# templeblock/audioSignalProcess

Hardware: AMD Instinct MI355X
Metric: audio frames/sec (10 ms @16 kHz) Wiener NS (higher is better)
Workload: dtype f32

## Files before the change

### audiosignalprocess_amd/csrc/ns_api.hip

```cpp
#include <hip/hip_runtime.h>

#include <chrono>

#include <math.h>
#include <stdio.h>
#include <stdlib.h>
#include <string.h>

#include <mutex>
#include <vector>

#include "api_common.h"
#include "asp_ns.h"
#include "handoff_host.h"
#include "ns_layout.h"

using namespace aspns;

namespace aspns {
hipError_t launch_ns_frame(int mode, float* state, int32_t* hist, const NsTables* T,
                           const float* in, float* out, int num_streams, hipStream_t s, bool g8 = false);
hipError_t launch_ns_frame1(bool io16, float* state, int32_t* hist, const NsTables* T,
                            const float* in, float* out, int num_streams, hipStream_t s, int steady_on,
                            unsigned long long* stamps = nullptr, int stamp_mode = 0, unsigned* step_counts = nullptr);
// ... 2 lines not shown
                                 unsigned* seq, unsigned* abort_w, unsigned want, int steps, int walk, int slot0,
                                 int ring, size_t per, int steady_on, unsigned long long* stamps = nullptr,
                                 unsigned* step_counts = nullptr);
hipError_t launch_ns_frame2(bool io16, float* state, int32_t* hist, const NsTables* T,
                            const float* in, float* out, int num_streams, hipStream_t s,
                            unsigned long long* stamps = nullptr);
hipError_t launch_ns_frame2_flow(bool io16, float* state, int32_t* hist, const NsTables* T,
                                 const float* in, float* out, int num_streams, hipStream_t s,
                                 unsigned* seq, unsigned* abort_w, unsigned want, int steps, int slot0, int ring,
                                 size_t per, unsigned long long* stamps = nullptr);
hipError_t launch_ns_unpair(float* state, int num_streams, hipStream_t s);
hipError_t launch_ns_hb_live(const float* state, const NsTables* T, const float* in_low,
                             int32_t* live, int num_streams, int hist_off, hipStream_t s);
hipError_t launch_ns_hb_apply(const float* state, float* hb_tail, const int32_t* live,
                              const NsTables* T, const float* in_high, float* out_high,
                              int num_streams, int num_high, int paired, hipStream_t s);
hipError_t launch_ns_set_policy(float* state, int num_streams, int mode, float overdrive,
                                float denoiseBound, int gainmap, hipStream_t s);
hipError_t launch_rdft256(float* data, int count, int isgn, const NsTables* T, hipStream_t s, int n = 256);
hipError_t launch_debug_eval(int fn, float* data, size_t n, const NsTables* T, hipStream_t s);
hipError_t launch_debug_tanh_wave(unsigned start, unsigned count, unsigned* n_bad, unsigned* bad_bits,
                                  const NsTables* T, hipStream_t s);
hipError_t launch_debug_guards_wave(unsigned start, unsigned count, unsigned* n_bad, unsigned* bad_bits, hipStream_t s);
hipError_t launch_debug_compare(int fn_a, int fn_b, unsigned start, unsigned count,
                                unsigned* n_bad, unsigned* bad_bits, float param,
                                const NsTables* T, hipStream_t s);
}

namespace {

#define fail(...) asp_fail(nullptr, __VA_ARGS__)
#define HIP_TRY(x) ASP_TRY(nullptr, x)
constexpr const char* kNoDevice = "no HIP device available (the NS engine has no CPU fallback)";


unsigned bitrev(unsigned x, int bits) {
  unsigned r = 0;
  for (int b = 0; b < bits; ++b) r |= ((x >> b) & 1u) << (bits - 1 - b);
  return r;
}

float window_entry(int i) {
  if (i >= 96 && i <= 160) return 1.0f;
  char buf[32];
  double s = sin(M_PI * (double)(i < 96 ? i : 256 - i) / 192.0);
  snprintf(buf, sizeof buf, "%.8f", s);
// ... 1460 lines not shown
  if (e == hipSuccess) e = hipMemcpy(data, d, n * sizeof(float), hipMemcpyDeviceToHost);
  (void)hipFree(d);
  if (e != hipSuccess) return fail(ASP_ERR_HIP, "debug_eval", e);
  return ASP_OK;
}

int AspNs_debug_compare(int fn_a, int fn_b, uint32_t start, uint32_t count, uint32_t* n_bad,
                        uint32_t* bad_bits64, float param, int device) {
  if (!n_bad || !bad_bits64) return fail(ASP_ERR_PARAM, "debug_compare: bad argument");
  AspDeviceScope dev_scope_;
  int rc = dev_scope_.select(nullptr, device, ASP_ERR_PARAM, kNoDevice);
  if (rc) return rc;
  NsTables* T = nullptr;
  rc = device_tables(device, &T);
  if (rc) return rc;
  unsigned* d = nullptr;
  HIP_TRY(hipMalloc((void**)&d, 65 * sizeof(unsigned)));
  hipError_t e = hipMemset(d, 0, 65 * sizeof(unsigned));
  if (e == hipSuccess && fn_a == 23 && fn_b != 3) e = hipErrorInvalidValue;
  if (e == hipSuccess && fn_a == 24 && fn_b != 9) e = hipErrorInvalidValue;
  if (e == hipSuccess)
    e = fn_a == 23   ? launch_debug_tanh_wave(start, count, d, d + 1, T, nullptr)
        : fn_a == 24 ? launch_debug_guards_wave(start, count, d, d + 1, nullptr)
                     : launch_debug_compare(fn_a, fn_b, start, count, d, d + 1, param, T, nullptr);
  unsigned h[65];
  if (e == hipSuccess) e = hipMemcpy(h, d, sizeof h, hipMemcpyDeviceToHost);
  (void)hipFree(d);
  if (e != hipSuccess) return fail(ASP_ERR_HIP, "debug_compare", e);
  *n_bad = h[0];
  memcpy(bad_bits64, h + 1, 64 * sizeof(unsigned));
  return ASP_OK;
}


struct NsHandleT {
  AspNsBatch* batch;
  int initFlag;
};

int WebRtcNs_Create(NsHandle** NS_inst) {
  if (!NS_inst) return -1;
  NsHandleT* h = (NsHandleT*)malloc(sizeof(NsHandleT));
  if (!h) return -1;
  h->batch = nullptr;
  h->initFlag = 0;
  if (AspNsBatch_Create(&h->batch, 1, 0) != ASP_OK) {
// ... 77 lines not shown
```

### audiosignalprocess_amd/csrc/ns_device.h

```cpp
#pragma once
#include <hip/hip_runtime.h>

namespace aspns_dev {

#ifdef NS1_BUDGET
#define ASP_NS_RARE(c) (__builtin_assume(!(c)), false)
#else
#define ASP_NS_RARE(c) __builtin_expect((c), 0)
#endif

__device__ __forceinline__ float xorf(float x, uint32_t m) {
  return __uint_as_float(__float_as_uint(x) ^ m);
}

__device__ __forceinline__ void wave_lds_fence() {
  __builtin_amdgcn_fence(__ATOMIC_RELEASE, "wavefront");
  __builtin_amdgcn_wave_barrier();
  __builtin_amdgcn_fence(__ATOMIC_ACQUIRE, "wavefront");
}

template <int CTRL>
__device__ __forceinline__ float dpp_move(float v) {
  return __int_as_float(__builtin_amdgcn_update_dpp(0, __float_as_int(v), CTRL, 0xF, 0xF, true));
}
// ... 56 lines not shown
  c = __int_as_float(__builtin_amdgcn_readlane(__float_as_int(c), 63));
  d = __int_as_float(__builtin_amdgcn_readlane(__float_as_int(d), 63));
}

__device__ __forceinline__ float div_by_uniform(float a, float d, float rd) {
  const float q0 = a * rd;
  const float r = __builtin_fmaf(-d, q0, a);
  return __builtin_fmaf(r, rd, q0);
}

__device__ __forceinline__ float fdiv_rcp(float d) {
  const float r0 = __builtin_amdgcn_rcpf(d);
  const float e0 = __builtin_fmaf(-d, r0, 1.0f);
  return __builtin_fmaf(e0, r0, r0);
}
__device__ __forceinline__ float fdiv_quot(float n, float d, float r1) {
  const float q0 = n * r1;
  const float e1 = __builtin_fmaf(-d, q0, n);
  const float q1 = __builtin_fmaf(e1, r1, q0);
  const float e2 = __builtin_fmaf(-d, q1, n);
  return __builtin_fmaf(e2, r1, q1);
}
__device__ __forceinline__ float fdiv(float n, float d) { return fdiv_quot(n, d, fdiv_rcp(d)); }
typedef float f32x2 __attribute__((ext_vector_type(2)));
__device__ __forceinline__ f32x2 fdiv2_rcp(f32x2 d) {
  f32x2 r0;
  r0.x = __builtin_amdgcn_rcpf(d.x);
  r0.y = __builtin_amdgcn_rcpf(d.y);
  const f32x2 one = {1.0f, 1.0f};
  const f32x2 e0 = __builtin_elementwise_fma(-d, r0, one);
  return __builtin_elementwise_fma(e0, r0, r0);
}
__device__ __forceinline__ f32x2 fdiv2_quot(f32x2 n, f32x2 d, f32x2 r1) {
  const f32x2 q0 = n * r1;
  const f32x2 e1 = __builtin_elementwise_fma(-d, q0, n);
  const f32x2 q1 = __builtin_elementwise_fma(e1, r1, q0);
  const f32x2 e2 = __builtin_elementwise_fma(-d, q1, n);
  return __builtin_elementwise_fma(e2, r1, q1);
}
__device__ __forceinline__ f32x2 fdiv2(f32x2 n, f32x2 d) { return fdiv2_quot(n, d, fdiv2_rcp(d)); }
struct B3 {
  bool v[3];
};
struct F3 {
  f32x2 p;
  float t;
  __device__ __forceinline__ F3() {}
  __device__ __forceinline__ F3(f32x2 p_, float t_) : p(p_), t(t_) {}
  __device__ __forceinline__ explicit F3(float c) : p(f32x2{c, c}), t(c) {}
  __device__ __forceinline__ explicit F3(const float (&x)[3]) : p(f32x2{x[0], x[1]}), t(x[2]) {}
  __device__ __forceinline__ void store(float (&x)[3]) const {
    x[0] = p.x; x[1] = p.y; x[2] = t;
  }
};
__device__ __forceinline__ F3 operator+(const F3& x, const F3& y) { return F3(x.p + y.p, x.t + y.t); }
__device__ __forceinline__ F3 operator-(const F3& x, const F3& y) { return F3(x.p - y.p, x.t - y.t); }
__device__ __forceinline__ F3 operator*(const F3& x, const F3& y) { return F3(x.p * y.p, x.t * y.t); }
__device__ __forceinline__ F3 operator*(float c, const F3& y) { return F3(c) * y; }
__device__ __forceinline__ F3 operator*(const F3& x, float c) { return x * F3(c); }
__device__ __forceinline__ F3 operator+(const F3& x, float c) { return x + F3(c); }
__device__ __forceinline__ F3 operator-(const F3& x, float c) { return x - F3(c); }
__device__ __forceinline__ F3 operator-(float c, const F3& y) { return F3(c) - y; }
__device__ __forceinline__ F3 fma3(const F3& x, const F3& y, const F3& z) {
// ... 119 lines not shown
  s = __builtin_fma(s0 * d, d, s);
  const double z = s * s;
  double p = 2.0 / 21.0;
  p = __builtin_fma(p, z, 2.0 / 19.0);
  p = __builtin_fma(p, z, 2.0 / 17.0);
  p = __builtin_fma(p, z, 2.0 / 15.0);
  p = __builtin_fma(p, z, 2.0 / 13.0);
  p = __builtin_fma(p, z, 2.0 / 11.0);
  p = __builtin_fma(p, z, 2.0 / 9.0);
  p = __builtin_fma(p, z, 2.0 / 7.0);
  p = __builtin_fma(p, z, 2.0 / 5.0);
  p = __builtin_fma(p, z, 2.0 / 3.0);
  const double lm = __builtin_fma(s * z, p, s + s);
  const double ed = (double)e;
  const double ln2_hi = 0x1.62e42fefa38p-1;
  const double ln2_lo = 0x1.ef35793c7673p-45;
  return __builtin_fma(ed, ln2_hi, __builtin_fma(ed, ln2_lo, lm));
}

__device__ __forceinline__ bool f64_rounds_safely_to_f32(double y) {
  const unsigned lo = (unsigned)__double2loint(y) & 0x1fffffffu;
  return ((lo - 0x0ffffe00u) > 0x400u);
}

__device__ __forceinline__ double exp_lean_f64(float xf, const double* __restrict__ t64) {
  const double x = (double)xf;
  const double kd = __builtin_rint(x * 0x1.71547652b82fep+6);
  const int k = (int)kd;
  double r = __builtin_fma(-kd, 0x1.62e42ff000000p-7, x);
  r = __builtin_fma(-kd, -0x1.718432a1b0e26p-41, r);
  double q = 1.0 / 120.0;
  q = __builtin_fma(q, r, 1.0 / 24.0);
  q = __builtin_fma(q, r, 1.0 / 6.0);
  q = __builtin_fma(q, r, 0.5);
  const double p = __builtin_fma(q, r * r, r);
  const double T = t64[k & 63];
  return __builtin_amdgcn_ldexp(__builtin_fma(T, p, T), k >> 6);
}

__device__ __forceinline__ float exp_f32_via_f64(float x, const double* __restrict__ t64) {
  const bool in_range = fabsf(x) <= 87.0f;
  const double y = exp_lean_f64(in_range ? x : 0.0f, t64);
  const bool ok = in_range && f64_rounds_safely_to_f32(y);
  float r = (float)y;
  if (ASP_NS_RARE(!ok)) r = (float)exp((double)x);
  return r;
// ... 5 lines not shown
  const double ad = (double)ax;
  const double a2 = ad * ad;
  double sr = 0x1.664f4882c10fap-6;
  sr = __builtin_fma(sr, a2, -0x1.ba1ba1ba1ba1cp-5);
  sr = __builtin_fma(sr, a2, 0x1.1111111111111p-3);
  sr = __builtin_fma(sr, a2, -0x1.5555555555555p-2);
  const double t_small = __builtin_fma(ad * a2, sr, ad);
  const double u = exp_lean_f64(finite_ok ? -2.0f * ax : 0.0f, t64);
  const double num = 1.0 - u, den = 1.0 + u;
  double rc = (double)__builtin_amdgcn_rcpf((float)den);
  rc = __builtin_fma(__builtin_fma(-den, rc, 1.0), rc, rc);
  rc = __builtin_fma(__builtin_fma(-den, rc, 1.0), rc, rc);
  double qv = num * rc;
  qv = __builtin_fma(__builtin_fma(-qv, den, num), rc, qv);
  const double t = ax < 0.03125f ? t_small : qv;
  const bool ok = finite_ok && f64_rounds_safely_to_f32(t);
  float r = __builtin_copysignf((float)t, a);
  if (ASP_NS_RARE(!ok)) r = (float)tanh((double)a);
  return r;
}

__device__ __forceinline__ float tanh_f32_via_f64_wave(float a, const double* __restrict__ t64) {
  const float ax = fabsf(a);
  const bool finite_ok = ax <= 40.0f;
  const double u = exp_lean_f64(finite_ok ? -2.0f * ax : 0.0f, t64);
  const double num = 1.0 - u, den = 1.0 + u;
  double rc = (double)__builtin_amdgcn_rcpf((float)den);
  rc = __builtin_fma(__builtin_fma(-den, rc, 1.0), rc, rc);
  double t = num * rc;
  t = __builtin_fma(__builtin_fma(-t, den, num), rc, t);
  const bool small = ax < 0.03125f;
  if (ASP_NS_RARE(__builtin_amdgcn_ballot_w64(small) != 0)) {
    const double ad = (double)ax;
    const double a2 = ad * ad;
    double sr = 0x1.664f4882c10fap-6;
    sr = __builtin_fma(sr, a2, -0x1.ba1ba1ba1ba1cp-5);
    sr = __builtin_fma(sr, a2, 0x1.1111111111111p-3);
    sr = __builtin_fma(sr, a2, -0x1.5555555555555p-2);
    const double t_small = __builtin_fma(ad * a2, sr, ad);
    t = small ? t_small : t;
  }
  const bool ok = finite_ok && f64_rounds_safely_to_f32(t);
  float r = __builtin_copysignf((float)t, a);
  if (ASP_NS_RARE(!ok)) r = (float)tanh((double)a);
  return r;
}

__device__ __forceinline__ float fsqrt(float x) {
  const float r = __builtin_amdgcn_rsqf(x);
  float g = x * r;
  float h = 0.5f * r;
  const float e = __builtin_fmaf(-h, g, 0.5f);
  g = __builtin_fmaf(g, e, g);
  h = __builtin_fmaf(h, e, h);
  const float d = __builtin_fmaf(-g, g, x);
  g = __builtin_fmaf(d, h, g);
  float res = (x == 0.0f || x == __builtin_inff()) ? x : g;
  if (ASP_NS_RARE(x < 0x1p-100f && x > 0.0f)) res = sqrtf(x);
  return res;
}

__device__ __forceinline__ float log_f32_via_f64(float x) {
  const unsigned ax = __float_as_uint(x);
  const bool normal_pos = (ax - 0x00800000u) < 0x7f000000u;
  const double y = log_lean_f64(x);
  const bool ok = normal_pos && f64_rounds_safely_to_f32(y);
  float r = (float)y;
// ... 41 lines not shown
#pragma unroll
  for (int k = 0; k < N; ++k) {
    const unsigned ax = __float_as_uint(x[k]);
    const unsigned normal_pos = (ax - 0x00800000u) < 0x7f000000u ? 1u : 0u;
    const double y = log_tab_f64(x[k], tab);
    bad |= (normal_pos ^ 1u) | (f64_rounds_safely_to_f32(y) ? 0u : 1u);
    out[k] = (float)y;
  }
  if (ASP_NS_RARE(bad != 0)) {
#pragma unroll
    for (int k = 0; k < N; ++k) out[k] = log_f32_slow(x[k]);
  }
}

template <int N>
__device__ __forceinline__ void exp_f32_via_f64_n(const float (&x)[N], float (&out)[N],
                                                  const double* __restrict__ t64) {
  unsigned bad = 0;
#pragma unroll
  for (int k = 0; k < N; ++k) {
    const unsigned in_range = fabsf(x[k]) <= 87.0f ? 1u : 0u;
    const double y = exp_lean_f64(x[k], t64);
    bad |= (in_range ^ 1u) | (f64_rounds_safely_to_f32(y) ? 0u : 1u);
    out[k] = (float)y;
  }
  if (ASP_NS_RARE(bad != 0)) {
#pragma unroll
    for (int k = 0; k < N; ++k) out[k] = exp_f32_slow(x[k]);
  }
}

template <int N>
__device__ __forceinline__ void fsqrt_n(const float (&x)[N], float (&out)[N]) {
  unsigned bad = 0;
#pragma unroll
  for (int k = 0; k < N; ++k) {
    const float xv = x[k];
    const float r = __builtin_amdgcn_rsqf(xv);
    float g = xv * r;
    float h = 0.5f * r;
    const float e = __builtin_fmaf(-h, g, 0.5f);
    g = __builtin_fmaf(g, e, g);
    h = __builtin_fmaf(h, e, h);
    const float d = __builtin_fmaf(-g, g, xv);
    g = __builtin_fmaf(d, h, g);
    out[k] = (xv == 0.0f || xv == __builtin_inff()) ? xv : g;
// ... 111 lines not shown
```

### audiosignalprocess_amd/csrc/ns_kernels1.hip

```cpp
#include <hip/hip_runtime.h>

#include <type_traits>

#include "handoff.h"
#include "ns_device.h"
#include "ns_layout.h"
#include "ns_pair_fft.h"
#include "ns_step.h"

namespace {
using namespace asphandoff;
using namespace aspns_dev;
using namespace aspns_pair;

__device__ __forceinline__ unsigned long long ns_cu_tag() {
  const unsigned hw = __builtin_amdgcn_s_getreg((7 << 11) | (8 << 6) | 4);
  const unsigned xcc = __builtin_amdgcn_s_getreg((3 << 11) | (0 << 6) | 20);
  return (unsigned long long)((xcc << 8) | hw);
}

constexpr int NS3 = 3;

template <typename V>
__device__ __forceinline__ V ns_in_vgpr(V x) {
// ... 214 lines not shown
      }                                                                                        \
      __builtin_amdgcn_sched_barrier(0);                                                       \
    }                                                                                          \
  }
#define NS_BUDGET_ASIDE()
#define NS_BUDGET_BACK(k)
#endif
  unsigned flow_j = 0, flow_end = 1, flow_slot = 0;
  [[maybe_unused]] unsigned diag_steps = 0;
  [[maybe_unused]] constexpr int ns_body_tag = 0;
  if constexpr (FLOW) {
    flow_j = blockIdx.y * fa.walk;
    flow_end = flow_j + fa.walk < fa.steps ? flow_j + fa.walk : fa.steps;
    flow_slot = ((unsigned)fa.slot0 + flow_j) % (unsigned)fa.ring;
  } else {
    NS_STAMP(0)
  }
  __shared__ __align__(16) float2 lds[4][130];
  __shared__ __align__(16) float tabs[3 * 64 * 4 + 32 * 4 * 2];
  __shared__ __align__(16) float wins[kAnal];
  __shared__ __align__(16) double exp2s[64];
  __shared__ __align__(16) double2 logts[128];
  __shared__ __align__(16) float imgs[FLOW ? 4 : 1][FLOW ? kImgDwords : 4];
  const int tid = threadIdx.x;
  const float4* tab_src = tid < 192 ? reinterpret_cast<const float4*>(&T->tw[0][0][0]) + tid
                                    : reinterpret_cast<const float4*>(&T->spl[0][0][0]) + (tid - 192);
  const float4 tab_v = *tab_src;
  const float4 win_v = reinterpret_cast<const float4*>(T->window)[tid & 63];
  const double exp2_v = T->exp2_64[tid & 63];
  const double2 logt_v = reinterpret_cast<const double2*>(T->logtab)[tid & 127];
  const int lane = tid & 63;
  const int diagbits = T->diag[lane];
  const int wv = __builtin_amdgcn_readfirstlane(tid >> 6);
  float2* tile = lds[wv];
  const int lam = lane >> 1, h = lane & 1;
  const int g = lam >> 4, q = lam & 15;
  const int binA = q + 64 * g + 16 * h;
  const uint32_t gmask = g ? 0x80000000u : 0u;
  const int stream_raw = blockIdx.x * 4 + wv;
  bool wave_live = stream_raw < num_streams;
  const int stream = wave_live ? stream_raw : num_streams - 1;
  float* __restrict__ st = state + (size_t)stream * kStreamDwords;
  int32_t* __restrict__ hist = hist_all + (size_t)stream * kHistDwords;
  const StateAcc<FLOW> sa(st, FLOW ? imgs[wv] : nullptr);
  float* outj = out;
  auto diag_flush_steps = [&]() __attribute__((always_inline)) {
    if constexpr (DIAG) {
      unsigned* const counts = reinterpret_cast<unsigned*>(diag_buf);
      if (dg.mode == 2 && ns_cold(lane) == 0) {
        atomicAdd(counts + 2 * stream, diag_steps & 0xffffu);
        atomicAdd(counts + 2 * stream + 1, diag_steps >> 16);
      }
    }
  };

  float sv;
  constexpr bool ROW_IMG = FLOW && !DIAG;
  const ScalarRow<ROW_IMG> srow(imgs[FLOW ? wv : 0]);
#define SC_I(k) __builtin_amdgcn_readlane(__float_as_int(sv), (k))
#define SC_F(k) srow.template f<(k)>(sv)
#define SC_SET_I(k, val) sv = writelane_bits<(k)>(sv, (int)(val))
#define SC_SET_F(k, val) srow.template set<(k)>(sv, (val))
  static_assert(S_COUNTER1 == S_COUNTER0 + 1 && S_COUNTER2 == S_COUNTER0 + 2, "the three counters: consecutive lanes");
  float4 s4;
  float2 carryA, carryB;
  float4 s4in = make_float4(0.f, 0.f, 0.f, 0.f);
  const size_t frame_uni = (size_t)stream * kBlockL;
  auto flow_load_in = [&](unsigned slot) __attribute__((always_inline)) {
    const int lane_c = ns_cold(lane);
    const unsigned frame_lane = 4u * (unsigned)((lane_c < 24 ? 24 : lane_c) - 24);
    const float* base = IO16 ? reinterpret_cast<const float*>(reinterpret_cast<const short*>(in + (size_t)slot * fa.per) + frame_uni)
                             : in + (size_t)slot * fa.per + frame_uni;
    s4in = load_frame4<IO16>(base, frame_lane);
  };
  auto flow_head = [&](auto head_c) __attribute__((always_inline)) {
// ... 20 lines not shown
      s4 = *reinterpret_cast<const float4*>(src);
    } else {
      const int lh = lane < 24 ? lane : 23, li = lane < 24 ? 24 : lane;
      const float4 ha = *reinterpret_cast<const float4*>(hbuf + 4 * lh);
      const short* in16 = reinterpret_cast<const short*>(in) + (size_t)stream * kBlockL + 4 * (li - 24);
      const short4 a = *reinterpret_cast<const short4*>(in16);
      const bool hsel = lane < 24;
      s4.x = hsel ? ha.x : (float)a.x;
      s4.y = hsel ? ha.y : (float)a.y;
      s4.z = hsel ? ha.z : (float)a.z;
      s4.w = hsel ? ha.w : (float)a.w;
    }
    carryA = *reinterpret_cast<const float2*>(st + kOffSynt + 2 * q + 32 * h);
    carryB = *reinterpret_cast<const float2*>(st + kOffSynt + 2 * q + 64);
  }

  reinterpret_cast<float4*>(tabs)[tid] = tab_v;
  if (tid < 64) exp2s[tid] = exp2_v;
  if (tid < 128) logts[tid] = logt_v;
  if (tid >= 192) reinterpret_cast<float4*>(wins)[tid - 192] = win_v;
  if constexpr (FLOW) {
    if (wave_live) sa.image_fill(lane, img_v);
  }
  __syncthreads();
  if (!wave_live) return;
  if constexpr (FLOW) {
    sv = sa.ld1(kOffScalars, lane);
    flow_head(std::integral_constant<int, 3>{});
  }
  const float* tws = tabs;
  const float* spls = tabs + 3 * 64 * 4;
  const PairFftLane fl = pair_fft_lane(lane, diagbits);

#define LOADV(dst, f)                                                                          \
  {                                                                                            \
    const float2 v2_ = sa.ld2(kOffVec + (f)*kVecStride, 2 * lane);                             \
    dst[0] = v2_.x; dst[1] = v2_.y;                                                            \
  }
#define LOADT(dst, f) dst[2] = SC_F(S_TAIL0 + (f));
#define LOAD3(dst, f) LOADV(dst, f) LOADT(dst, f)
#define STORE3(f, srcv)                                                                        \
  {                                                                                            \
    sa.st2(kOffVec + (f)*kVecStride, 2 * lane, srcv[0], srcv[1]);                              \
    SC_SET_F(S_TAIL0 + (f), srcv[2]);                                                          \
  }
#define STORE3_HOT(f, srcv)                                                                    \
  {                                                                                            \
    sa.st2(kOffVec + (f)*kVecStride, 2 * lane, srcv[0], srcv[1]);                              \
    if constexpr (!ROW_IMG) SC_SET_F(S_TAIL0 + (f), srcv[2]);                                  \
  }
#define NS_NEXT_FRAME()                                                                        \
  if constexpr (FLOW) {                                                                        \
    flow_slot = flow_slot + 1u == (unsigned)fa.ring ? 0u : flow_slot + 1u;                     \
    if (flow_j + 1u < flow_end) flow_load_in(flow_slot);                                       \
  }
#define NS_STREAM_DONE(head_tag)                                                               \
  if constexpr (FLOW) {                                                                        \
    [[maybe_unused]] constexpr int ns_body_tag = head_tag;  \
    const bool walk_done_ = flow_j + 1u >= flow_end;                                           \
    if (walk_done_) {                                                                          \
      NS_BUDGET_ASIDE()                                                                        \
      const int lane_w_ = ns_cold(lane);                                                       \
      srow.store_owned(lane_w_, sv);                                                           \
      lds_sync1();                                                                             \
      sa.image_write_back(lane_w_);                                                            \
      handoff_drain();                                                                         \
    }                                                                                          \
    NS_STAMP(16)                                                                               \
    if (walk_done_) {                                                                          \
      NS_BUDGET_ASIDE()                                                                        \
      diag_flush_steps();                                                                      \
      if (lane == 0) handoff_publish(fa.hand.seq + stream, fa.want + flow_j);                  \
      return;                                                                                  \
    }                                                                                          \
    ++flow_j;                                                                                  \
    lds_sync1();                                                                               \
    NS_BUDGET_BACK(16)                                                                         \
    flow_head(std::integral_constant<int, head_tag>{});                                        \
    continue;                                                                                  \
  } else {                                                                                     \
    diag_flush_steps();                                                                        \
    return;                                                                                    \
  }

  constexpr bool CARRY = FLOW;
  [[maybe_unused]] f32x2 carry_stsa = {0.f, 0.f};
  [[maybe_unused]] float carry_stsa_tail = 0.f;
// ... 131 lines not shown
        } else {
          const float q1t = fdiv(magnPrevA[2], noisePrev[2] + 0.0001f);
          previousEstimateStsa = q1t * smooth[2];
        }
        prevStsa[2] = previousEstimateStsa;
        snrLocPost[2] = 0.f;
        if (magn[2] > noise2) snrLocPost[2] = q2t - 1.f;
        snrLocPrior[2] = NS_DD_PR_SNR * previousEstimateStsa + (1.f - NS_DD_PR_SNR) * snrLocPost[2];
      };
      auto load_snr_tails = [&]() __attribute__((always_inline)) {
        static_assert(V_SMOOTH == V_QUANT + 1 && V_MAGNPREV_A == V_NOISEPREV + 1, "row tails read as pairs");
        float t2[2], u2[2];
        srow.template ld<S_TAIL0 + V_QUANT, 2>(sv, t2);
        srow.template ld<S_TAIL0 + V_NOISEPREV, 2>(sv, u2);
        quant[2] = t2[0]; smooth[2] = t2[1];
        noisePrev[2] = u2[0]; magnPrevA[2] = u2[1];
      };
      float lmagn[NS3];
      [[maybe_unused]] float lt1_tail = 0.f;
      if constexpr (STEADY) {
        load_snr_tails();
        snr_tail(quant[2]);
        const float xs[NS3] = {magn[0], magn[1], lane == 1 ? 1.f + 2.f * snrLocPrior[2] : magn[2]};
        log_f32_via_tab_n<NS3>(xs, lmagn, logts);
        lt1_tail = lane_bcast(lmagn[2], 1);
        lmagn[2] = lane_bcast(lmagn[2], 0);
      } else {
        log_f32_via_tab_n<NS3>(magn, lmagn, logts);
      }
      LOADT(avgPause, V_AVGPAUSE)

      NS_STAMP(3)
      float signalEnergy, sumMagn, flatNum, avgPauseMean;
      {
        float p_se = (re[0] * re[0] + im[0] * im[0]) + (re[1] * re[1] + im[1] * im[1]);
        float p_sm = magn[0] + magn[1];
        float p_fl = lane == 0 ? lmagn[1] : lmagn[0] + lmagn[1];
        float p_ap = avgPause[0] + avgPause[1];
        wave_sums_bcast(p_se, p_sm, p_fl, p_ap);
        signalEnergy = p_se + (re[2] * re[2] + im[2] * im[2]);
        sumMagn = p_sm + magn[2];
        flatNum = p_fl + lmagn[2];
        avgPauseMean = p_ap + avgPause[2];
        signalEnergy = DIV129(signalEnergy);
      }

      NS_STAMP(4)
      if constexpr (!STEADY) load_snr_tails();
      if (updates < NS_END_STARTUP_LONG) updates++;
      bool quant_new = false;
      constexpr int kLqLane = S_TAIL0 + V_LQ0, kDenLane = S_TAIL0 + V_DEN0;
// ... 1 lines not shown
                    kDenLane == kLqLane + 3 && kLqLane / 16 == (kDenLane + 2) / 16,
                    "the tracker tails: three + three consecutive lanes of one DPP row");
      float lqT = sv, denT = dpp_move<0x103>(sv);
      {
#define NS_LANES3_F(j) __int_as_float(lanes3_bits<kLqLane>(__float_as_int(cterm[0][j]), __float_as_int(cterm[1][j]), \
                                                           __float_as_int(cterm[2][j])))
        const float cntv = NS_LANES3_F(0), cnt1v = NS_LANES3_F(1), rcnt1v = NS_LANES3_F(2);
#undef NS_LANES3_F
        tracker_step1(lqT, denT, lmagn[2], cntv, cnt1v, rcnt1v);
      }
#pragma unroll
      for (int s = 0; s < 3; ++s) {
        {
          const float cnt = cterm[s][0], cnt1 = cterm[s][1], rcnt1 = cterm[s][2];
          f32x2 lq = {LQ[s][0], LQ[s][1]}, den = {DEN[s][0], DEN[s][1]};
          tracker_step2(lq, den, f32x2{lmagn[0], lmagn[1]}, cnt, cnt1, rcnt1);
          LQ[s][0] = lq.x; LQ[s][1] = lq.y;
          DEN[s][0] = den.x; DEN[s][1] = den.y;
        }
        if (counter[s] >= NS_END_STARTUP_LONG) {
          counter[s] = 0;
          if (updates >= NS_END_STARTUP_LONG) {
            LQ[s][2] = lane_bcast(lqT, kLqLane + s);
            exp_f32_via_f64_n<NS3>(LQ[s], quant, exp2s);
            quant_new = true;
          }
        }
        counter[s]++;
      }
      if (updates < NS_END_STARTUP_LONG) {
        LQ[2][2] = lane_bcast(lqT, kLqLane + 2);
        exp_f32_via_f64_n<NS3>(LQ[2], quant, exp2s);
        quant_new = true;
      }
#pragma unroll
      for (int k = 0; k < NS3; ++k) noise[k] = quant[k];
#pragma unroll
      for (int s = 0; s < 3; ++s) sa.st2(kOffVec + (V_LQ0 + s) * kVecStride, 2 * lane, LQ[s][0], LQ[s][1]);
#pragma unroll
      for (int s = 0; s < 3; ++s) sa.st2(kOffVec + (V_DEN0 + s) * kVecStride, 2 * lane, DEN[s][0], DEN[s][1]);
      sv = mergelanes_vgpr<(7ull << kLqLane)>(sv, lqT);
      sv = mergelanes_vgpr<(7ull << kDenLane)>(sv, dpp_move<0x113>(denT));
      if (quant_new) STORE3(V_QUANT, quant)

      NS_STAMP(5)
      float whiteNoiseLevel = SC_F(S_WHITE);
      float pinkNoiseNumerator = SC_F(S_PINKNUM);
      float pinkNoiseExp = SC_F(S_PINKEXP);
      float fd5, fd6;
      {
        static_assert(S_FD6 == S_FD5 + 1, "read as a pair");
        float t2[2];
        srow.template ld<S_FD5, 2>(sv, t2);
        fd5 = t2[0]; fd6 = t2[1];
      }
// ... 108 lines not shown
        varPause += vp[2];
        varMagn += vm[2];
        covMagnPause = DIV129(covMagnPause);
        varPause = DIV129(varPause);
        varMagn = DIV129(varMagn);
        fd6 += signalEnergy;
        diffa = ns_spectral_diff_args(covMagnPause, varPause, fd5);
        diff_varMagn = varMagn;
      }

      NS_STAMP(8)
      {
        float t1[NS3], lt1[NS3];
        LOADT(logLrt, V_LOGLRT)
#pragma unroll
        for (int k = 0; k < NS3; ++k) t1[k] = 1.f + 2.f * snrLocPrior[k];
        if constexpr (STEADY) {
          const float t1p[2] = {t1[0], t1[1]};
          float lt1p[2];
          log_f32_via_tab_n<2>(t1p, lt1p, logts);
          lt1[0] = lt1p[0]; lt1[1] = lt1p[1];
          lt1[2] = lt1_tail;
        } else {
          log_f32_via_tab_n<NS3>(t1, lt1, logts);
        }
        float tn[NS3], td3[NS3], t2v[NS3];
#pragma unroll
        for (int k = 0; k < NS3; ++k) {
          tn[k] = 2.f * snrLocPrior[k];
          td3[k] = t1[k] + 0.0001f;
        }
        {
          const f32x2 a = fdiv2(f32x2{tn[0], tn[1]}, f32x2{td3[0], td3[1]});
          const f32x2 b = fdiv2(f32x2{tn[2], diffa.n1}, f32x2{td3[2], diffa.d1});
          t2v[0] = a.x; t2v[1] = a.y; t2v[2] = b.x;
          diffa.n1 = diff_varMagn - b.y;
        }
#pragma unroll
        for (int k = 0; k < NS3; ++k) {
          const float t2 = t2v[k];
          const float besselTmp = (snrLocPost[k] + 1.f) * t2;
          logLrt[k] += NS_LRT_TAVG * (besselTmp - lt1[k] - logLrt[k]);
        }
      }
      float logLrtTimeAvgKsum = SUM3(logLrt);
      logLrtTimeAvgKsum = DIV129(logLrtTimeAvgKsum);
      float ev[NS3], fd0 = SC_F(S_FD0), fd3 = SC_F(S_FD3), pmp2;
      {
        float t4[4];
        srow.template ld<S_PMP0, 4>(sv, t4);
        pm.p0 = t4[0]; pm.p1 = t4[1]; pmp2 = t4[2]; pm.p3 = t4[3];
        pm.p4 = pm.p5 = pm.p6 = 0.f;
      }
      {
        float nl[NS3];
#pragma unroll
        for (int k = 0; k < NS3; ++k) nl[k] = -logLrt[k];
        nl[2] = lane == 0 ? flat.arg : nl[2];
        exp_f32_via_f64_n<NS3>(nl, ev, exp2s);
        {
          const f32x2 qq = fdiv2(f32x2{lane_bcast(ev[2], 0), diffa.n1}, f32x2{flat.den, diffa.d2});
          fd0 = ns_flatness_update_q(fd0, qq.x);
          fd4 = ns_spectral_diff_q(fd4, qq.y);
        }
        ev[2] = lane_bcast(ev[2], 1);
      }

      NS_STAMP(9)
      int mup0 = updateParsFlag, mup3 = ss.mup3;
      const int mup1 = SC_I(S_MUP1);
      bool window_closed = false;
      if (updateParsFlag >= 1) {
        mup3--;
        if (mup3 > 0) {
          const int lane_c = ns_cold(lane);
          const float fv = lane_c == 0 ? fd3 : (lane_c == 1 ? fd0 : fd4);
          const float bw = lane_c == 1 ? 0.05f : 0.1f, rbw = lane_c == 1 ? 1.0f / 0.05f : 1.0f / 0.1f;
          const float lim = lane_c == 1 ? kHist * 0.05f : kHist * 0.1f;
          if (lane_c < 3 && (fv < lim) && (fv >= 0.0f))
            atomicAdd(&hist[lane_c * kHistStride + (int)div_by_uniform(fv, bw, rbw)], 1);
        }
        if (mup3 == 0) {
          if constexpr (FLOW) handoff_drain();
          pm = close_histogram_window<FLOW>(hist, lane, mup1, mup0 >= 1, pm);
          if constexpr (FLOW) handoff_drain();
          window_closed = true;
          const NsWindowOpen wo = ns_window_reopen(updateParsFlag, mup1, fd5, fd6);
          mup0 = wo.mup0;
          mup3 = wo.mup3;
          fd5 = wo.fd5;
          fd6 = wo.fd6;
        }
      }
      fd3 = logLrtTimeAvgKsum;
      {
// ... 7 lines not shown
        const float widthPrior0 = NS_WIDTH_PR_MAP, widthPrior1 = 2.f * NS_WIDTH_PR_MAP,
                    widthPrior2 = 2.f * NS_WIDTH_PR_MAP;
        const int sgnMap = (int)pmp2;
        float widthPrior = widthPrior0;
        if (logLrtTimeAvgKsum < pm.p0) widthPrior = widthPrior1;
        const float arg0 = widthPrior * (logLrtTimeAvgKsum - pm.p0);
        widthPrior = widthPrior0;
        if (sgnMap == 1 && (fd0 > pm.p1)) widthPrior = widthPrior1;
        if (sgnMap == -1 && (fd0 < pm.p1)) widthPrior = widthPrior1;
        const float arg1 = (float)sgnMap * widthPrior * (pm.p1 - fd0);
        widthPrior = widthPrior0;
        if (fd4 < pm.p3) widthPrior = widthPrior2;
        const float arg2 = widthPrior * (fd4 - pm.p3);
        const float arg = lane == 0 ? arg0 : (lane == 1 ? arg1 : arg2);
        const float th = tanh_f32_via_f64_wave(arg, exp2s);
        priorSpeechProb = ns_prior_update(priorSpeechProb, pm, ns_prior_indicator(lane_bcast(th, 0)),
                                          ns_prior_indicator(lane_bcast(th, 1)), ns_prior_indicator(lane_bcast(th, 2)));
      }
      float probSpeech[NS3];
      {
        const float gainPrior = fdiv(1.f - priorSpeechProb, priorSpeechProb + 0.0001f);
        {
          float pd[NS3];
          const float ones[NS3] = {1.f, 1.f, 1.f};
#pragma unroll
          for (int k = 0; k < NS3; ++k) {
            float invLrt = ev[k];
            invLrt = (float)gainPrior * invLrt;
            pd[k] = 1.f + invLrt;
          }
          fdiv3(ones, pd, probSpeech);
        }
      }

      NS_STAMP(10)
      {
        const int srcA = q > 0 ? lane - 2 : (h ? 30 + 32 * g : 31);
        const int srcB = q > 0 ? lane - 2 : (h ? 30 + 32 * g : 31 + 32 * g);
        const bool a_from1 = q == 0 && h == 0;
        const bool b_from1 = q > 0 || h == 1;
        const float a0 = __shfl(probSpeech[0], srcA, 64), a1 = __shfl(probSpeech[1], srcA, 64);
        const float b0 = __shfl(probSpeech[0], srcB, 64), b1 = __shfl(probSpeech[1], srcB, 64);
        float prevProb[NS3];
        prevProb[0] = a_from1 ? a1 : a0;
        prevProb[1] = b_from1 ? b1 : b0;
        prevProb[2] = lane_bcast(probSpeech[1], 63);
        {
          const F3 np(noisePrev), mg(magn), ps(probSpeech), ap(avgPause);
          const F3 x = (1.f - ps) * mg + ps * np;
          const F3 uS = NS_SPEECH_UPDATE * np + (1.f - NS_SPEECH_UPDATE) * x;
          const F3 uN = NS_NOISE_UPDATE * np + (1.f - NS_NOISE_UPDATE) * x;
          B3 oldSpeech = gt3(F3(prevProb), F3(NS_PROB_RANGE));
          oldSpeech.v[0] = oldSpeech.v[0] && lane != 0;
          const F3 uOld = sel3(oldSpeech, uS, uN);
// ... 241 lines not shown
  const float a = tanh_f32_via_f64_wave(x, T->exp2_64), b = (float)tanh((double)x);
  const bool same = (__float_as_uint(a) == __float_as_uint(b)) || (a != a && b != b);
  if (!same) {
    const unsigned k = atomicAdd(n_bad, 1u);
    if (k < 64) bad_bits[k] = start + i;
  }
}

__global__ void debug_guards_wave_kernel(unsigned start, unsigned count, unsigned* n_bad, unsigned* bad_bits) {
  const unsigned i = blockIdx.x * blockDim.x + threadIdx.x;
  if (i >= count) return;
  const float x = __uint_as_float(start + i);
  float emitted = x;
  if (__builtin_amdgcn_ballot_w64(sat16p_may_clip(x)) != 0) emitted = sat16p(x);
  const float a = fsqrt_wave(x), b = sqrtf(x);
  const bool same = __float_as_uint(emitted) == __float_as_uint(sat16p(x)) &&
                    ((__float_as_uint(a) == __float_as_uint(b)) || (a != a && b != b));
  if (!same) {
    const unsigned k = atomicAdd(n_bad, 1u);
    if (k < 64) bad_bits[k] = start + i;
  }
}

}

namespace aspns {

hipError_t launch_debug_guards_wave(unsigned start, unsigned count, unsigned* n_bad, unsigned* bad_bits, hipStream_t s) {
  hipLaunchKernelGGL(debug_guards_wave_kernel, dim3((count + 255u) / 256u), dim3(256), 0, s, start, count, n_bad, bad_bits);
  return hipGetLastError();
}

hipError_t launch_debug_tanh_wave(unsigned start, unsigned count, unsigned* n_bad, unsigned* bad_bits,
                                  const NsTables* T, hipStream_t s) {
  hipLaunchKernelGGL(debug_tanh_wave_kernel, dim3((count + 255u) / 256u), dim3(256), 0, s, start, count, n_bad, bad_bits, T);
  return hipGetLastError();
}

hipError_t launch_ns_frame1(bool io16, float* state, int32_t* hist, const NsTables* T,
                            const float* in, float* out, int num_streams, hipStream_t s, int steady_on,
                            unsigned long long* stamps, int stamp_mode, unsigned* step_counts) {
  const dim3 grid((num_streams + 3) / 4), block(256);
  const NsFlowArgs none = {{nullptr, nullptr}, 0u, 0, 1, 0u, 1u, 1u};
  if (stamps != nullptr || step_counts != nullptr) {
    if (io16) return hipErrorInvalidValue;
    const NsDiagArgs dg = {stamps != nullptr ? (void*)stamps : (void*)step_counts, stamps != nullptr ? (stamp_mode != 0 ? 1 : 0) : 2};
    hipLaunchKernelGGL((ns_frame1_diag_kernel<false>), grid, block, 0, s, state, hist, T, in, out, num_streams,
                       steady_on, none, dg);
  } else if (io16)
// ... 33 lines not shown
```

### audiosignalprocess_amd/csrc/ns_step.h

```cpp
#pragma once
#include <hip/hip_runtime.h>

#include "ns_device.h"
#include "ns_layout.h"

namespace aspns_dev {
using namespace aspns;

#define NS_QUANTILE (float)0.25
#define NS_END_STARTUP_LONG 200
#define NS_END_STARTUP_SHORT 50
#define NS_FACTOR (float)40.0
#define NS_WIDTH (float)0.01
#define NS_DD_PR_SNR (float)0.98
#define NS_LRT_TAVG (float)0.50
#define NS_SPECT_FL_TAVG (float)0.30
#define NS_SPECT_DIFF_TAVG (float)0.30
#define NS_PRIOR_UPDATE (float)0.10
#define NS_NOISE_UPDATE (float)0.90
#define NS_SPEECH_UPDATE (float)0.99
#define NS_WIDTH_PR_MAP (float)4.0
#define NS_PROB_RANGE (float)0.20
#define NS_GAMMA_PAUSE (float)0.05
#define NS_B_LIM (float)0.5
// ... 232 lines not shown
    fd6 = 0.f;
  }
  return {mup0, mup1, fd5, fd6};
}

__device__ __forceinline__ float ns_prior_indicator(float th) { return 0.5f * (th + 1.f); }
__device__ __forceinline__ float ns_prior_update(float priorSpeechProb, PriorModel pm, float indicator0,
                                                 float indicator1, float indicator2) {
  const float indPrior = pm.p4 * indicator0 + pm.p5 * indicator1 + pm.p6 * indicator2;
  priorSpeechProb += NS_PRIOR_UPDATE * (indPrior - priorSpeechProb);
  if (priorSpeechProb > 1.f) priorSpeechProb = 1.f;
  if (priorSpeechProb < 0.01f) priorSpeechProb = 0.01f;
  return priorSpeechProb;
}

template <bool WAVE_SQRT = false>
__device__ __forceinline__ float ns_gain_factor(float energy2, float energy1, float denoiseBound,
                                                float priorSpeechProb) {
  float factor1 = 1.f, factor2 = 1.f;
  const float ratio = fdiv(energy2, energy1 + 1.f);
  float gain = WAVE_SQRT ? fsqrt_wave(ratio) : fsqrt(ratio);
  if (gain > NS_B_LIM) {
    factor1 = 1.f + 1.3f * (gain - NS_B_LIM);
    if (gain * factor1 > 1.f) factor1 = fdiv(1.f, gain);
  }
  if (gain < NS_B_LIM) {
    if (gain <= denoiseBound) gain = denoiseBound;
    factor2 = 1.f - 0.3f * (NS_B_LIM - gain);
  }
  return priorSpeechProb * factor1 + (1.f - priorSpeechProb) * factor2;
}

}
```

Baseline: 492.6 million.

## Defer histogram atomics into an LDS ring and use wave-uniform fallback guards

In steady-state flow mode, the per-step feature histogram updates are written to a small per-wave LDS ring of 8 steps. They are flushed with atomics in batches, and the flush replaces an existing LDS sync point instead of being issued every step. Log and exp fallback checks now use wave ballots and a cheaper unsafe-rounding test, so the slow path is chosen once per wave. Reciprocal-only divisions are replaced with a shorter frcp/frcp2 sequence. This cuts per-step atomics, sync and divergent-branch overhead, at the cost of delaying histogram updates and adding more LDS state and a new debug kernel.

Result: faster. 505.2 million, median of 6 (+2.5%).

```diff
diff --git a/audiosignalprocess_amd/csrc/ns_api.hip b/audiosignalprocess_amd/csrc/ns_api.hip
--- a/audiosignalprocess_amd/csrc/ns_api.hip
+++ b/audiosignalprocess_amd/csrc/ns_api.hip
@@ -48,6 +48,8 @@
 hipError_t launch_debug_tanh_wave(unsigned start, unsigned count, unsigned* n_bad, unsigned* bad_bits,
                                   const NsTables* T, hipStream_t s);
 hipError_t launch_debug_guards_wave(unsigned start, unsigned count, unsigned* n_bad, unsigned* bad_bits, hipStream_t s);
+hipError_t launch_debug_fallbacks_wave(int what, unsigned start, unsigned count, unsigned* n_bad, unsigned* bad_bits,
+                                       const NsTables* T, hipStream_t s);
 hipError_t launch_debug_compare(int fn_a, int fn_b, unsigned start, unsigned count,
                                 unsigned* n_bad, unsigned* bad_bits, float param,
                                 const NsTables* T, hipStream_t s);
@@ -1554,6 +1556,7 @@
   if (e == hipSuccess)
     e = fn_a == 23   ? launch_debug_tanh_wave(start, count, d, d + 1, T, nullptr)
         : fn_a == 24 ? launch_debug_guards_wave(start, count, d, d + 1, nullptr)
+        : fn_a == 25 ? launch_debug_fallbacks_wave(fn_b, start, count, d, d + 1, T, nullptr)
                      : launch_debug_compare(fn_a, fn_b, start, count, d, d + 1, param, T, nullptr);
   unsigned h[65];
   if (e == hipSuccess) e = hipMemcpy(h, d, sizeof h, hipMemcpyDeviceToHost);
diff --git a/audiosignalprocess_amd/csrc/ns_device.h b/audiosignalprocess_amd/csrc/ns_device.h
--- a/audiosignalprocess_amd/csrc/ns_device.h
+++ b/audiosignalprocess_amd/csrc/ns_device.h
@@ -102,6 +102,11 @@
   return __builtin_fmaf(e2, r1, q1);
 }
 __device__ __forceinline__ float fdiv(float n, float d) { return fdiv_quot(n, d, fdiv_rcp(d)); }
+__device__ __forceinline__ float frcp(float d) {
+  const float r1 = fdiv_rcp(d);
+  const float e1 = __builtin_fmaf(-d, r1, 1.0f);
+  return __builtin_fmaf(e1, r1, r1);
+}
 typedef float f32x2 __attribute__((ext_vector_type(2)));
 __device__ __forceinline__ f32x2 fdiv2_rcp(f32x2 d) {
   f32x2 r0;
@@ -119,6 +124,12 @@
   return __builtin_elementwise_fma(e2, r1, q1);
 }
 __device__ __forceinline__ f32x2 fdiv2(f32x2 n, f32x2 d) { return fdiv2_quot(n, d, fdiv2_rcp(d)); }
+__device__ __forceinline__ f32x2 frcp2(f32x2 d) {
+  const f32x2 one = {1.0f, 1.0f};
+  const f32x2 r1 = fdiv2_rcp(d);
+  const f32x2 e1 = __builtin_elementwise_fma(-d, r1, one);
+  return __builtin_elementwise_fma(e1, r1, r1);
+}
 struct B3 {
   bool v[3];
 };
@@ -284,6 +295,10 @@
   const unsigned lo = (unsigned)__double2loint(y) & 0x1fffffffu;
   return ((lo - 0x0ffffe00u) > 0x400u);
 }
+__device__ __forceinline__ bool f64_lo_rounds_unsafely(unsigned lo) { return ((lo << 3) - 0x7ffff000u) <= 0x2000u; }
+__device__ __forceinline__ bool f64_rounds_unsafely_to_f32(double y) {
+  return f64_lo_rounds_unsafely((unsigned)__double2loint(y));
+}
 
 __device__ __forceinline__ double exp_lean_f64(float xf, const double* __restrict__ t64) {
   const double x = (double)xf;
@@ -335,8 +350,8 @@
 
 __device__ __forceinline__ float tanh_f32_via_f64_wave(float a, const double* __restrict__ t64) {
   const float ax = fabsf(a);
-  const bool finite_ok = ax <= 40.0f;
-  const double u = exp_lean_f64(finite_ok ? -2.0f * ax : 0.0f, t64);
+  const unsigned long long far = __builtin_amdgcn_ballot_w64(!(ax <= 40.0f));
+  const double u = exp_lean_f64(-2.0f * ax, t64);
   const double num = 1.0 - u, den = 1.0 + u;
   double rc = (double)__builtin_amdgcn_rcpf((float)den);
   rc = __builtin_fma(__builtin_fma(-den, rc, 1.0), rc, rc);
@@ -353,9 +368,9 @@
     const double t_small = __builtin_fma(ad * a2, sr, ad);
     t = small ? t_small : t;
   }
-  const bool ok = finite_ok && f64_rounds_safely_to_f32(t);
+  const unsigned long long bad = far | __builtin_amdgcn_ballot_w64(f64_rounds_unsafely_to_f32(t));
   float r = __builtin_copysignf((float)t, a);
-  if (ASP_NS_RARE(!ok)) r = (float)tanh((double)a);
+  if (ASP_NS_RARE(bad != 0)) r = (float)tanh((double)a);
   return r;
 }
 
@@ -443,6 +458,45 @@
     const unsigned in_range = fabsf(x[k]) <= 87.0f ? 1u : 0u;
     const double y = exp_lean_f64(x[k], t64);
     bad |= (in_range ^ 1u) | (f64_rounds_safely_to_f32(y) ? 0u : 1u);
+    out[k] = (float)y;
+  }
+  if (ASP_NS_RARE(bad != 0)) {
+#pragma unroll
+    for (int k = 0; k < N; ++k) out[k] = exp_f32_slow(x[k]);
+  }
+}
+
+__device__ __forceinline__ unsigned long long lanes_not_positive_normal(float x) {
+  unsigned long long m;
+  asm("v_cmp_class_f32_e64 %0, %1, %2" : "=s"(m) : "v"(x), "s"(0x3ffu & ~0x100u));
+  return m;
+}
+template <int N>
+__device__ __forceinline__ void log_f32_via_tab_n_wave(const float (&x)[N], float (&out)[N],
+                                                       const double2* __restrict__ tab) {
+  unsigned long long bad = 0;
+#pragma unroll
+  for (int k = 0; k < N; ++k) {
+    bad |= lanes_not_positive_normal(x[k]);
+    const double y = log_tab_f64(x[k], tab);
+    bad |= __builtin_amdgcn_ballot_w64(f64_rounds_unsafely_to_f32(y));
+    out[k] = (float)y;
+  }
+  if (ASP_NS_RARE(bad != 0)) {
+#pragma unroll
+    for (int k = 0; k < N; ++k) out[k] = log_f32_slow(x[k]);
+  }
+}
+
+template <int N>
+__device__ __forceinline__ void exp_f32_via_f64_n_wave(const float (&x)[N], float (&out)[N],
+                                                       const double* __restrict__ t64) {
+  unsigned long long bad = 0;
+#pragma unroll
+  for (int k = 0; k < N; ++k) {
+    bad |= __builtin_amdgcn_ballot_w64(!(fabsf(x[k]) <= 87.0f));
+    const double y = exp_lean_f64(x[k], t64);
+    bad |= __builtin_amdgcn_ballot_w64(f64_rounds_unsafely_to_f32(y));
     out[k] = (float)y;
   }
   if (ASP_NS_RARE(bad != 0)) {
diff --git a/audiosignalprocess_amd/csrc/ns_kernels1.hip b/audiosignalprocess_amd/csrc/ns_kernels1.hip
--- a/audiosignalprocess_amd/csrc/ns_kernels1.hip
+++ b/audiosignalprocess_amd/csrc/ns_kernels1.hip
@@ -260,6 +260,9 @@
   __shared__ __align__(16) double exp2s[64];
   __shared__ __align__(16) double2 logts[128];
   __shared__ __align__(16) float imgs[FLOW ? 4 : 1][FLOW ? kImgDwords : 4];
+  constexpr bool DEFER = FLOW && !DIAG;
+  constexpr int kPendSteps = 8, kPendLanes = 3 * kPendSteps;
+  __shared__ __align__(16) float pends[DEFER ? 4 : 1][DEFER ? kPendLanes : 1];
   const int tid = threadIdx.x;
   const float4* tab_src = tid < 192 ? reinterpret_cast<const float4*>(&T->tw[0][0][0]) + tid
                                     : reinterpret_cast<const float4*>(&T->spl[0][0][0]) + (tid - 192);
@@ -289,6 +292,24 @@
         atomicAdd(counts + 2 * stream, diag_steps & 0xffffu);
         atomicAdd(counts + 2 * stream + 1, diag_steps >> 16);
       }
+    }
+  };
+
+  lds_f32* const pend = (lds_f32*)pends[DEFER ? wv : 0];
+  auto hist_flush = [&]() __attribute__((always_inline)) {
+    if constexpr (DEFER) {
+      const int lane_c = ns_cold(lane);
+      lds_sync1();
+      if (lane_c < kPendLanes) {
+        const float fv = pend[lane_c];
+        pend[lane_c] = -1.f;
+        const int f = lane_c % 3;
+        const float bw = f == 1 ? 0.05f : 0.1f, rbw = f == 1 ? 1.0f / 0.05f : 1.0f / 0.1f;
+        const float lim = f == 1 ? kHist * 0.05f : kHist * 0.1f;
+        if ((fv < lim) && (fv >= 0.0f))
+          atomicAdd(&hist[f * kHistStride + (int)div_by_uniform(fv, bw, rbw)], 1);
+      }
+      lds_sync1();
     }
   };
 
@@ -355,6 +376,9 @@
   if constexpr (FLOW) {
     if (wave_live) sa.image_fill(lane, img_v);
   }
+  if constexpr (DEFER) {
+    if (lane < kPendLanes) pends[wv][lane] = -1.f;
+  }
   __syncthreads();
   if (!wave_live) return;
   if constexpr (FLOW) {
@@ -395,7 +419,8 @@
       NS_BUDGET_ASIDE()                                                                        \
       const int lane_w_ = ns_cold(lane);                                                       \
       srow.store_owned(lane_w_, sv);                                                           \
-      lds_sync1();                                                                             \
+      hist_flush();       \
+      if constexpr (!DEFER) lds_sync1();                                                       \
       sa.image_write_back(lane_w_);                                                            \
       handoff_drain();                                                                         \
     }                                                                                          \
@@ -573,11 +598,11 @@
         load_snr_tails();
         snr_tail(quant[2]);
         const float xs[NS3] = {magn[0], magn[1], lane == 1 ? 1.f + 2.f * snrLocPrior[2] : magn[2]};
-        log_f32_via_tab_n<NS3>(xs, lmagn, logts);
+        log_f32_via_tab_n_wave<NS3>(xs, lmagn, logts);
         lt1_tail = lane_bcast(lmagn[2], 1);
         lmagn[2] = lane_bcast(lmagn[2], 0);
       } else {
-        log_f32_via_tab_n<NS3>(magn, lmagn, logts);
+        log_f32_via_tab_n_wave<NS3>(magn, lmagn, logts);
       }
       LOADT(avgPause, V_AVGPAUSE)
 
@@ -625,7 +650,7 @@
           counter[s] = 0;
           if (updates >= NS_END_STARTUP_LONG) {
             LQ[s][2] = lane_bcast(lqT, kLqLane + s);
-            exp_f32_via_f64_n<NS3>(LQ[s], quant, exp2s);
+            exp_f32_via_f64_n_wave<NS3>(LQ[s], quant, exp2s);
             quant_new = true;
           }
         }
@@ -633,7 +658,7 @@
       }
       if (updates < NS_END_STARTUP_LONG) {
         LQ[2][2] = lane_bcast(lqT, kLqLane + 2);
-        exp_f32_via_f64_n<NS3>(LQ[2], quant, exp2s);
+        exp_f32_via_f64_n_wave<NS3>(LQ[2], quant, exp2s);
         quant_new = true;
       }
 #pragma unroll
@@ -788,7 +813,7 @@
           lt1[0] = lt1p[0]; lt1[1] = lt1p[1];
           lt1[2] = lt1_tail;
         } else {
-          log_f32_via_tab_n<NS3>(t1, lt1, logts);
+          log_f32_via_tab_n_wave<NS3>(t1, lt1, logts);
         }
         float tn[NS3], td3[NS3], t2v[NS3];
 #pragma unroll
@@ -823,7 +848,7 @@
 #pragma unroll
         for (int k = 0; k < NS3; ++k) nl[k] = -logLrt[k];
         nl[2] = lane == 0 ? flat.arg : nl[2];
-        exp_f32_via_f64_n<NS3>(nl, ev, exp2s);
+        exp_f32_via_f64_n_wave<NS3>(nl, ev, exp2s);
         {
           const f32x2 qq = fdiv2(f32x2{lane_bcast(ev[2], 0), diffa.n1}, f32x2{flat.den, diffa.d2});
           fd0 = ns_flatness_update_q(fd0, qq.x);
@@ -836,7 +861,16 @@
       int mup0 = updateParsFlag, mup3 = ss.mup3;
       const int mup1 = SC_I(S_MUP1);
       bool window_closed = false;
-      if (updateParsFlag >= 1) {
+      if constexpr (DEFER && !STEADY) hist_flush();
+      if constexpr (STEADY && DEFER) {
+        const unsigned rel = flow_j - blockIdx.y * fa.walk;
+        if (rel >= (unsigned)kPendSteps) hist_flush();
+        mup3--;
+        if (lane == 0) {
+          lds_f32* const slot = pend + 3 * (rel & (kPendSteps - 1));
+          slot[0] = fd3; slot[1] = fd0; slot[2] = fd4;
+        }
+      } else if (updateParsFlag >= 1) {
         mup3--;
         if (mup3 > 0) {
           const int lane_c = ns_cold(lane);
@@ -890,14 +924,15 @@
         const float gainPrior = fdiv(1.f - priorSpeechProb, priorSpeechProb + 0.0001f);
         {
           float pd[NS3];
-          const float ones[NS3] = {1.f, 1.f, 1.f};
 #pragma unroll
           for (int k = 0; k < NS3; ++k) {
             float invLrt = ev[k];
             invLrt = (float)gainPrior * invLrt;
             pd[k] = 1.f + invLrt;
           }
-          fdiv3(ones, pd, probSpeech);
+          const f32x2 ps2 = frcp2(f32x2{pd[0], pd[1]});
+          probSpeech[0] = ps2.x; probSpeech[1] = ps2.y;
+          probSpeech[2] = frcp(pd[2]);
         }
       }
 
@@ -1185,9 +1220,65 @@
   }
 }
 
+__global__ void debug_fallbacks_wave_kernel(int what, unsigned start, unsigned count, unsigned* n_bad,
+                                            unsigned* bad_bits, const NsTables* __restrict__ T) {
+  const unsigned i = blockIdx.x * blockDim.x + threadIdx.x;
+  const bool live = i < count;
+  const unsigned bits = start + (live ? i : 0u);
+  const float x = __uint_as_float(bits);
+  const double2* lt = reinterpret_cast<const double2*>(T->logtab);
+  auto eq = [](float a, float b) { return (__float_as_uint(a) == __float_as_uint(b)) || (a != a && b != b); };
+  bool same = true;
+  if (what == 0) {
+    const unsigned lo = bits & 0x1fffffffu;
+    same = f64_lo_rounds_unsafely(bits) == !((lo - 0x0ffffe00u) > 0x400u);
+  } else if (what == 1) {
+    const float want = fdiv(1.f, x);
+    const f32x2 a = frcp2(f32x2{x, 1.5f}), b = frcp2(f32x2{3.f, x});
+    same = __float_as_uint(frcp(x)) == __float_as_uint(want) && __float_as_uint(a.x) == __float_as_uint(want) &&
+           __float_as_uint(b.y) == __float_as_uint(want) && __float_as_uint(a.y) == __float_as_uint(fdiv(1.f, 1.5f)) &&
+           __float_as_uint(b.x) == __float_as_uint(fdiv(1.f, 3.f));
+  } else if (what == 2 || what == 4) {
+    const bool is_log = what == 2;
+    const float benign = is_log ? 1.5f : 0.5f;
+    const float want = is_log ? log_f32_via_tab(x, lt) : exp_f32_via_f64(x, T->exp2_64);
+    const float want_benign = is_log ? log_f32_via_tab(benign, lt) : exp_f32_via_f64(benign, T->exp2_64);
+    const int lane = threadIdx.x & 63;
+    for (int j = 0; j < 64; ++j) {
+      const float in[1] = {lane == j ? x : benign};
+      float o[1];
+      if (is_log) log_f32_via_tab_n_wave<1>(in, o, lt);
+      else exp_f32_via_f64_n_wave<1>(in, o, T->exp2_64);
+      same = same && eq(o[0], lane == j ? want : want_benign);
+    }
+  } else if (what == 3) {
+    const float in[1] = {x};
+    float o[1];
+    log_f32_via_tab_n_wave<1>(in, o, lt);
+    same = eq(o[0], log_f32_via_tab(x, lt));
+  } else {
+    const float in[1] = {x};
+    float o[1];
+    exp_f32_via_f64_n_wave<1>(in, o, T->exp2_64);
+    same = eq(o[0], exp_f32_via_f64(x, T->exp2_64));
+  }
+  if (live && !same) {
+    const unsigned k = atomicAdd(n_bad, 1u);
+    if (k < 64) bad_bits[k] = bits;
+  }
+}
+
 }
 
 namespace aspns {
+
+hipError_t launch_debug_fallbacks_wave(int what, unsigned start, unsigned count, unsigned* n_bad, unsigned* bad_bits,
+                                       const NsTables* T, hipStream_t s) {
+  if (what < 0 || what > 5) return hipErrorInvalidValue;
+  hipLaunchKernelGGL(debug_fallbacks_wave_kernel, dim3((count + 255u) / 256u), dim3(256), 0, s, what, start, count,
+                     n_bad, bad_bits, T);
+  return hipGetLastError();
+}
 
 hipError_t launch_debug_guards_wave(unsigned start, unsigned count, unsigned* n_bad, unsigned* bad_bits, hipStream_t s) {
   hipLaunchKernelGGL(debug_guards_wave_kernel, dim3((count + 255u) / 256u), dim3(256), 0, s, start, count, n_bad, bad_bits);
diff --git a/audiosignalprocess_amd/csrc/ns_step.h b/audiosignalprocess_amd/csrc/ns_step.h
--- a/audiosignalprocess_amd/csrc/ns_step.h
+++ b/audiosignalprocess_amd/csrc/ns_step.h
@@ -278,7 +278,7 @@
   float gain = WAVE_SQRT ? fsqrt_wave(ratio) : fsqrt(ratio);
   if (gain > NS_B_LIM) {
     factor1 = 1.f + 1.3f * (gain - NS_B_LIM);
-    if (gain * factor1 > 1.f) factor1 = fdiv(1.f, gain);
+    if (gain * factor1 > 1.f) factor1 = WAVE_SQRT ? frcp(gain) : fdiv(1.f, gain);
   }
   if (gain < NS_B_LIM) {
     if (gain <= denoiseBound) gain = denoiseBound;
```
